# llm-d-incubation/workload-variant-autoscaler

Measured on AMD Instinct MI355X. Metric: solver_wall_clock_ms, lower is better.
Workload: dtype fp64; 1 GPU; model=3 models x 2 service classes (config #3), variants=64, accelerator_types=3, global_batch=64, seq_len=0, parallelism=fleet-shard dp1, analyzer_device=cuda

## Files before the change

### wva_amd/csrc/queue_core.h

```cpp
#pragma once

#include <cmath>

#if defined(__HIPCC__)
#define WVA_HD __host__ __device__ inline
#else
#define WVA_HD inline
#endif

namespace wva {

constexpr double kEpsilon = 0.001;
constexpr double kStabilityFraction = 0.1;
constexpr double kTolerance = 1e-6;
constexpr int kMaxIterations = 100;
constexpr int kMaxQueueToBatchRatio = 10;

enum ProblemField {
  P_ALPHA = 0,
  P_BETA,
  P_GAMMA,
  P_DELTA,
  P_IN_TOKENS,
  P_OUT_TOKENS,
  P_MAX_BATCH,
  P_TARGET_TTFT,
  P_TARGET_ITL,
  P_TARGET_TPS,
  P_TOTAL_RATE,
  P_MIN_REPLICAS,
  PROBLEM_FIELDS
};

enum ResultField {
  R_FEASIBLE = 0,
  R_REPLICAS,
  R_RATE_STAR,
  R_ITL,
  R_TTFT,
  R_RHO,
  RESULT_FIELDS
};

struct Parms {
  double alpha, beta, gamma, delta;
  double in_tokens;
  int out_tokens;
  int max_batch;
  int num_decode;
  double wait_scale;
};

constexpr int kMaxBatchLimit = 2147483647 / (1 + kMaxQueueToBatchRatio);

WVA_HD bool row_valid(const double *pr, double scv = 1.0) {
  bool ok = (scv >= 0.0) & (scv <= 1.7976931348623157e308);
  for (int f = 0; f < PROBLEM_FIELDS; ++f) {
    ok &= fabs(pr[f]) <= 1.7976931348623157e308;
  }
  ok &= (pr[P_ALPHA] >= 0.0) & (pr[P_BETA] >= 0.0) & (pr[P_GAMMA] >= 0.0) &
        (pr[P_DELTA] >= 0.0);
  ok &= (pr[P_MAX_BATCH] >= 1.0) & (pr[P_MAX_BATCH] < (double)kMaxBatchLimit + 1.0);
  ok &= (pr[P_OUT_TOKENS] >= 1.0) & (pr[P_OUT_TOKENS] < 2147483648.0);
  ok &= pr[P_IN_TOKENS] >= 0.0;
  ok &= (pr[P_TARGET_TTFT] >= 0.0) & (pr[P_TARGET_ITL] >= 0.0) & (pr[P_TARGET_TPS] >= 0.0);
  return ok;
}

WVA_HD Parms parms_from_problem(const double *pr, double scv = 1.0) {
  Parms p;
  p.alpha = pr[P_ALPHA];
  p.beta = pr[P_BETA];
  p.gamma = pr[P_GAMMA];
  p.delta = pr[P_DELTA];
  p.in_tokens = trunc(pr[P_IN_TOKENS]);
  p.out_tokens = (int)pr[P_OUT_TOKENS];
  p.max_batch = (int)pr[P_MAX_BATCH];
  p.num_decode = p.out_tokens - 1;
  if (p.in_tokens == 0.0 && p.out_tokens == 1) p.num_decode = 1;
  p.wait_scale = (1.0 + scv) / 2.0;
  return p;
}

WVA_HD int row_chain_length(const double *pr) {
  return row_valid(pr) ? (int)pr[P_MAX_BATCH] * (1 + kMaxQueueToBatchRatio) : 0;
}

WVA_HD double prefill_time(const Parms &p, double batch) {
  return p.in_tokens == 0.0 ? 0.0 : p.gamma + p.delta * p.in_tokens * batch;
}

WVA_HD double decode_time(const Parms &p, double batch) {
  return p.alpha + p.beta * batch;
}

WVA_HD double serv_rate(const Parms &p, int b) {
  return (double)b / (prefill_time(p, (double)b) + p.num_decode * decode_time(p, (double)b));
}

WVA_HD double log_mu(const Parms &p, int n) {
  int b = n + 1;
  if (b > p.max_batch) b = p.max_batch;
  return log(serv_rate(p, b));
}

WVA_HD bool within_tolerance(double x, double value, double tolerance) {
  if (x == value) return true;
  if (value == 0.0 || tolerance < 0.0) return false;
  return fabs((x - value) / value) <= tolerance;
}

WVA_HD double effective_concurrency(const Parms &p, double avg_serv_time) {
  double tokens = (double)(p.out_tokens - 1);
  double numer = avg_serv_time - (p.gamma + p.alpha * tokens);
  double denom = p.delta * p.in_tokens + p.beta * tokens;
  if (denom == 0.0) return numer > 0.0 ? (double)p.max_batch : 0.0;
  double n = numer / denom;
  if (n < 0.0) n = 0.0;
  if (n > (double)p.max_batch) n = (double)p.max_batch;
  return n;
}

struct Stats {
  double throughput;
  double wait;
  double serv;
  double n_serv;
};

WVA_HD bool rate_below(const Parms &p, int b, double lam) {
  double t = prefill_time(p, (double)b) + p.num_decode * decode_time(p, (double)b);
  return (double)b < lam * t;
}

WVA_HD int log_mode_state(const Parms &p, int K, double lam) {
  double tN = prefill_time(p, (double)p.max_batch) +
              p.num_decode * decode_time(p, (double)p.max_batch);
  if ((double)p.max_batch <= lam * tN) return K;
  double t1 = prefill_time(p, 1.0) + p.num_decode * decode_time(p, 1.0);
  if (lam * t1 <= 1.0) return 0;
  int lo = 1, hi = p.max_batch;
  while (lo < hi) {
    int mid = (lo + hi) / 2;
    if (rate_below(p, mid, lam)) {
      lo = mid + 1;
    } else {
      hi = mid;
    }
  }
  return lo - 1;
}

WVA_HD double log_p(const double *cum, double loglam, int n) {
  return (n == 0) ? 0.0 : n * loglam - cum[n - 1];
}

constexpr double kLogCutoff = 45.0;

WVA_HD void state_window(const double *cum, double loglam, int K, int n_star,
                         double m, int *lo_out, int *hi_out) {
  const double thresh = m - kLogCutoff;
  int lo = 0, hi = n_star;
  while (lo < hi) {
    int mid = (lo + hi) / 2;
    if (log_p(cum, loglam, mid) < thresh) {
      lo = mid + 1;
    } else {
      hi = mid;
    }
  }
  *lo_out = lo;
  lo = n_star;
  hi = K;
  while (lo < hi) {
    int mid = (lo + hi + 1) / 2;
    if (log_p(cum, loglam, mid) < thresh) {
      hi = mid - 1;
    } else {
      lo = mid;
    }
  }
  *hi_out = lo;
}

struct GeoTail {
  double S, Ni, eK;
  bool used;
};

WVA_HD GeoTail geo_tail(double x_a, double d, int g_start, int n_hi, int K) {
  GeoTail t{0.0, 0.0, 0.0, false};
  const int M = n_hi - g_start;
  if (M < 8 || fabs(d) * (double)(M + 1) < 0.01) return t;
  const double p_a = exp(x_a);
  const double e1 = expm1(d);
  const double G0 = expm1((double)(M + 1) * d) / e1;
  const double r = e1 + 1.0;
  const double rM = exp((double)M * d);
  const double G1 =
      r * (1.0 - (double)(M + 1) * rM + (double)M * rM * r) / (e1 * e1);
  t.S = p_a * G0;
  t.Ni = p_a * ((double)g_start * G0 + G1);
  if (n_hi == K) t.eK = p_a * exp((double)(K - g_start) * d);
  t.used = true;
  return t;
}

WVA_HD Stats stats_of_sums(double lam, int num, double S, double Ni, double Snum,
                           double Ninum, double eK) {
  Stats st;
  st.throughput = lam * (1.0 - eK / S);
  double n_sys = Ni / S;
  st.n_serv = Ninum / S + (1.0 - Snum / S) * (double)num;
  if (st.throughput == 0.0) {
    st.wait = st.serv = 0.0;
  } else {
    double resp = n_sys / st.throughput;
    st.serv = st.n_serv / st.throughput;
    st.wait = resp - st.serv;
    if (st.wait < 0.0) st.wait = 0.0;
  }
  return st;
}

WVA_HD Stats eval_model(const Parms &p, const double *cum, int K, double lam) {
  double loglam = log(lam);
  int n_star = log_mode_state(p, K, lam);
  double m = log_p(cum, loglam, n_star);
  if (m < 0.0) m = 0.0;
  int n_lo, n_hi;
  state_window(cum, loglam, K, n_star, m, &n_lo, &n_hi);
  int num = p.max_batch;
  double S = 0.0, Ni = 0.0, Snum = 0.0, Ninum = 0.0, eK = 0.0;
  const int g_start = (num + 1 > n_lo) ? num + 1 : n_lo;
  GeoTail tail{0.0, 0.0, 0.0, false};
  int loop_hi = n_hi;
  if (g_start + 8 <= n_hi) {
    const double d = loglam - (cum[g_start] - cum[g_start - 1]);
    tail = geo_tail(log_p(cum, loglam, g_start) - m, d, g_start, n_hi, K);
    if (tail.used) loop_hi = g_start - 1;
  }
  for (int n = n_lo; n <= loop_hi; ++n) {
    double e = exp(log_p(cum, loglam, n) - m);
    S += e;
    Ni += n * e;
    if (n <= num) {
      Snum += e;
      Ninum += n * e;
    }
    if (n == K) eK = e;
  }
  S += tail.S;
  Ni += tail.Ni;
  eK += tail.eK;
  return stats_of_sums(lam, num, S, Ni, Snum, Ninum, eK);
}


WVA_HD double cum_at(const double *cum, int N, double log_mu_n, int n) {
  const int i = n < N ? n : N - 1;
  const double base = cum[i];
  return n < N ? base : base + (double)(n - N + 1) * log_mu_n;
}

WVA_HD double log_p_compact(const double *cum, int N, double log_mu_n, double loglam,
                            int n) {
  return (n == 0) ? 0.0 : n * loglam - cum_at(cum, N, log_mu_n, n - 1);
}

WVA_HD GeoTail geo_tail_compact(const double *cum, int N, double log_mu_n, double loglam,
                                double m, int *loop_hi) {
  const int K = N * (1 + kMaxQueueToBatchRatio);
  const int g_start = N + 1;
  const double d = loglam - log_mu_n;
  const GeoTail tail = geo_tail(
      log_p_compact(cum, N, log_mu_n, loglam, g_start) - m, d, g_start, K, K);
  *loop_hi = tail.used ? N : K;
  return tail;
}

WVA_HD Stats eval_model_compact(const Parms &p, const double *cum, double log_mu_n,
                                double lam) {
  const int num = p.max_batch;
  const int K = num * (1 + kMaxQueueToBatchRatio);
  const double loglam = log(lam);
  const int n_star = log_mode_state(p, K, lam);
  double m = log_p_compact(cum, num, log_mu_n, loglam, n_star);
  if (m < 0.0) m = 0.0;
  int loop_hi;
  const GeoTail tail = geo_tail_compact(cum, num, log_mu_n, loglam, m, &loop_hi);
  double S = 0.0, Ni = 0.0, Snum = 0.0, Ninum = 0.0, eK = 0.0;
  for (int n = 0; n <= loop_hi; ++n) {
    double e = exp(log_p_compact(cum, num, log_mu_n, loglam, n) - m);
    S += e;
    Ni += n * e;
    if (n <= num) {
      Snum += e;
      Ninum += n * e;
    }
    if (n == K) eK = e;
  }
  S += tail.S;
  Ni += tail.Ni;
  eK += tail.eK;
  return stats_of_sums(lam, num, S, Ni, Snum, Ninum, eK);
}

WVA_HD double eval_ttft_of(const Parms &p, const Stats &st) {
  double effc = effective_concurrency(p, st.serv);
  return st.wait * p.wait_scale + prefill_time(p, effc);
}

WVA_HD double eval_itl_of(const Parms &p, const Stats &st) {
  double effc = effective_concurrency(p, st.serv);
  return decode_time(p, effc);
}


constexpr int kBisect = 2;

WVA_HD int classify_bracket(double x_min, double x_max, double y0, double y1,
                            double y_target, double *x_star, bool *increasing) {
  if (within_tolerance(y0, y_target, kTolerance)) {
    *x_star = x_min;
    return 0;
  }
  if (within_tolerance(y1, y_target, kTolerance)) {
    *x_star = x_max;
    return 0;
  }
  if (within_tolerance(y0, y1, kTolerance)) {
    if (y_target > fmax(y0, y1)) {
      *x_star = x_max;
      return +1;
    }
    *x_star = x_min;
    return -1;
  }
  *increasing = y0 < y1;
  if ((*increasing && y_target < y0) || (!*increasing && y_target > y0)) {
    *x_star = x_min;
    return -1;
  }
  if ((*increasing && y_target > y1) || (!*increasing && y_target < y1)) {
    *x_star = x_max;
    return +1;
  }
  return kBisect;
}

template <typename F>
WVA_HD int binary_search(double x_min, double x_max, double y_target, F eval,
                         double *x_star) {
  const double y0 = eval(x_min);
  const double y1 = eval(x_max);
  bool increasing = false;
  const int ind = classify_bracket(x_min, x_max, y0, y1, y_target, x_star, &increasing);
  if (ind != kBisect) return ind;
  double xs = x_min;
  for (int i = 0; i < kMaxIterations; ++i) {
    xs = 0.5 * (x_min + x_max);
    double ys = eval(xs);
    if (within_tolerance(ys, y_target, kTolerance)) break;
    if ((increasing && y_target < ys) || (!increasing && y_target > ys)) {
      x_max = xs;
    } else {
      x_min = xs;
    }
  }
  *x_star = xs;
  return 0;
}


WVA_HD void rate_bracket(const Parms &p, double *lam_min, double *lam_max) {
  *lam_min = serv_rate(p, 1) * kEpsilon;
  *lam_max = serv_rate(p, p.max_batch) * (1.0 - kEpsilon);
}

template <typename Ev>
WVA_HD bool search_targets(const double *pr, const Parms &p, const Ev &ev, double lam_min,
                           double lam_max, double *lam_ttft, double *lam_itl) {
  *lam_ttft = lam_max;
  if (pr[P_TARGET_TTFT] > 0.0) {
    auto ttft = [&](double lam) { return eval_ttft_of(p, ev.eval(lam)); };
    if (binary_search(lam_min, lam_max, pr[P_TARGET_TTFT], ttft, lam_ttft) < 0) return false;
  }
  *lam_itl = lam_max;
  if (pr[P_TARGET_ITL] > 0.0) {
    auto itl = [&](double lam) { return eval_itl_of(p, ev.eval(lam)); };
    if (binary_search(lam_min, lam_max, pr[P_TARGET_ITL], itl, lam_itl) < 0) return false;
  }
  return true;
}

struct RowValues {
  double feasible, replicas, rate_star, itl, ttft, rho;
};

template <typename Ev>
WVA_HD RowValues row_tail(const double *pr, const Parms &p, const Ev &ev, double lam_max,
                          double lam_ttft, double lam_itl) {
  double lam_tps = lam_max;
  if (pr[P_TARGET_TPS] > 0.0) lam_tps = lam_max * (1.0 - kStabilityFraction);

  const double lam = fmin(lam_ttft, fmin(lam_itl, lam_tps));
  Stats st = ev.eval(lam);
  const double rate_star = st.throughput * 1000.0;

  const double total_rate = pr[P_TOTAL_RATE];
  double n_rep = ceil(total_rate / rate_star);
  const double min_rep = trunc(pr[P_MIN_REPLICAS]);
  if (n_rep < min_rep) n_rep = min_rep;
  if (!(n_rep > 0.0)) return RowValues{};
  const double rate = total_rate / n_rep;
  if (!(rate > 0.0) || rate > lam_max * 1000.0) return RowValues{};

  Stats fin = ev.eval(rate / 1000.0);
  double rho = fin.n_serv / (double)p.max_batch;
  rho = fmin(fmax(rho, 0.0), 1.0);

  return RowValues{1.0, n_rep, rate_star, eval_itl_of(p, fin), eval_ttft_of(p, fin), rho};
}

template <typename Ev>
WVA_HD RowValues solve_row(const double *pr, const Parms &p, const Ev &ev) {
  double lam_min, lam_max, lam_ttft, lam_itl;
  rate_bracket(p, &lam_min, &lam_max);
  if (!search_targets(pr, p, ev, lam_min, lam_max, &lam_ttft, &lam_itl)) return RowValues{};
  return row_tail(pr, p, ev, lam_max, lam_ttft, lam_itl);
}

}
```

### wva_amd/csrc/queue_solver_hip.hip

```cpp

#include <hip/hip_runtime.h>

#include "queue_core.h"

namespace wva {



template <typename Pred>
__device__ inline int wave_lower_bound(int lo, int hi, int lane, Pred pred) {
  while (hi - lo >= 64) {
    const int step = (hi - lo + 63) >> 6;
    const int i = lo + lane * step;
    const bool t = (i >= hi) ? true : pred(i);
    const unsigned long long mask = __ballot(t);
    if (mask == 0ull) {
      lo = lo + 63 * step + 1;
      continue;
    }
    const int first = __ffsll((long long)mask) - 1;
    if (first == 0) return lo;
    lo = lo + (first - 1) * step + 1;
    const int cap = lo - 1 + step;
    if (cap < hi) hi = cap;
  }
  const int i = lo + lane;
  const bool t = (i >= hi) ? true : pred(i);
  const unsigned long long mask = __ballot(t);
  return lo + __ffsll((long long)mask) - 1;
}


struct LdsFullTable {
  const double *cum;
  int K;
  static __device__ bool fits(const double *pr, int max_k) {
    return row_chain_length(pr) <= max_k;
  }
  __device__ LdsFullTable(const Parms &p, const double *table)
      : cum(table), K(p.max_batch * (1 + kMaxQueueToBatchRatio)) {}
  __device__ int scan_length() const { return K; }
  __device__ int chain() const { return K; }
  __device__ double log_p(double loglam, int n) const { return wva::log_p(cum, loglam, n); }
  __device__ GeoTail tail(int num, double loglam, double m, int *loop_hi) const {
    const int g_start = num + 1;
    GeoTail t{0.0, 0.0, 0.0, false};
    *loop_hi = K;
    if (g_start + 8 <= K) {
      const double d = loglam - (cum[g_start] - cum[g_start - 1]);
      t = geo_tail(log_p(loglam, g_start) - m, d, g_start, K, K);
      if (t.used) *loop_hi = g_start - 1;
    }
    return t;
  }
};

struct LdsCompactTable {
  const double *cum;
  int N;
  double log_mu_n;
  static __device__ bool fits(const double *pr, int max_n) {
    return trunc(pr[P_MAX_BATCH]) <= (double)max_n;
  }
  __device__ LdsCompactTable(const Parms &p, const double *table)
      : cum(table), N(p.max_batch), log_mu_n(log_mu(p, p.max_batch - 1)) {}
  __device__ int scan_length() const { return N; }
  __device__ int chain() const { return N * (1 + kMaxQueueToBatchRatio); }
  __device__ double log_p(double loglam, int n) const {
    return log_p_compact(cum, N, log_mu_n, loglam, n);
  }
  __device__ GeoTail tail(int, double loglam, double m, int *loop_hi) const {
    return geo_tail_compact(cum, N, log_mu_n, loglam, m, loop_hi);
  }
};

template <int THREADS, typename Table>
struct WgEval {
  static constexpr int WAVES = THREADS / 64;
  const Parms &p;
  Table table;
  double *red;

  __device__ int mode_state_wave(int K, double lam, int lane) const {
    double tN = prefill_time(p, (double)p.max_batch) +
                p.num_decode * decode_time(p, (double)p.max_batch);
    if ((double)p.max_batch <= lam * tN) return K;
    double t1 = prefill_time(p, 1.0) + p.num_decode * decode_time(p, 1.0);
    if (lam * t1 <= 1.0) return 0;
    const int b = wave_lower_bound(
        1, p.max_batch, lane, [&](int i) { return !rate_below(p, i, lam); });
    return b - 1;
  }

  __device__ Stats eval(double lam) const {
    const int tid = threadIdx.x;
    const int wave = tid >> 6;
    const int lane = tid & 63;
    const int K = table.chain();
    const double loglam = log(lam);

    int n_star;
    if constexpr (WAVES == 1) {
      n_star = mode_state_wave(K, lam, lane);
    } else {
      n_star = log_mode_state(p, K, lam);
    }
    double m = table.log_p(loglam, n_star);
    if (m < 0.0) m = 0.0;
    if constexpr (WAVES > 1) {
      __syncthreads();
    }

    const int num = p.max_batch;
    const int idx = (WAVES == 1) ? lane : tid;
    int loop_hi;
    const GeoTail tail = table.tail(num, loglam, m, &loop_hi);
    double S = 0.0, Ni = 0.0, Snum = 0.0, Ninum = 0.0, eK = 0.0;
    {
      double S1 = 0.0, Ni1 = 0.0, Snum1 = 0.0, Ninum1 = 0.0, eK1 = 0.0;
      int n = idx;
      for (; n + THREADS <= loop_hi; n += 2 * THREADS) {
        const int n2 = n + THREADS;
        const double e = exp(table.log_p(loglam, n) - m);
        const double e2 = exp(table.log_p(loglam, n2) - m);
        S += e;
        Ni += (double)n * e;
        S1 += e2;
        Ni1 += (double)n2 * e2;
        if (n <= num) {
          Snum += e;
          Ninum += (double)n * e;
        }
        if (n2 <= num) {
          Snum1 += e2;
          Ninum1 += (double)n2 * e2;
        }
        if (n == K) eK = e;
        if (n2 == K) eK1 = e2;
      }
      if (n <= loop_hi) {
        const double e = exp(table.log_p(loglam, n) - m);
        S += e;
        Ni += (double)n * e;
        if (n <= num) {
          Snum += e;
          Ninum += (double)n * e;
        }
        if (n == K) eK = e;
      }
      S += S1;
      Ni += Ni1;
      Snum += Snum1;
      Ninum += Ninum1;
      eK += eK1;
    }
    for (int off = 32; off > 0; off >>= 1) {
      S += __shfl_down(S, off, 64);
      Ni += __shfl_down(Ni, off, 64);
      Snum += __shfl_down(Snum, off, 64);
      Ninum += __shfl_down(Ninum, off, 64);
      eK += __shfl_down(eK, off, 64);
    }
    if constexpr (WAVES == 1) {
      S = __shfl(S, 0, 64);
      Ni = __shfl(Ni, 0, 64);
      Snum = __shfl(Snum, 0, 64);
      Ninum = __shfl(Ninum, 0, 64);
      eK = __shfl(eK, 0, 64);
    } else {
      if (lane == 0) {
        red[wave * 5 + 0] = S;
        red[wave * 5 + 1] = Ni;
        red[wave * 5 + 2] = Snum;
        red[wave * 5 + 3] = Ninum;
        red[wave * 5 + 4] = eK;
      }
      __syncthreads();
      S = Ni = Snum = Ninum = eK = 0.0;
      for (int w = 0; w < WAVES; ++w) {
        S += red[w * 5 + 0];
        Ni += red[w * 5 + 1];
        Snum += red[w * 5 + 2];
        Ninum += red[w * 5 + 3];
        eK += red[w * 5 + 4];
      }
    }
    S += tail.S;
    Ni += tail.Ni;
    eK += tail.eK;
    return stats_of_sums(lam, num, S, Ni, Snum, Ninum, eK);
  }
};

__device__ inline double row_scv(const double *scv, int pid) {
  return scv != nullptr ? scv[pid] : 1.0;
}

template <typename Table>
__device__ inline bool row_rejected(const double *pr, double scv, int reserved) {
  return !(row_valid(pr, scv) & Table::fits(pr, reserved));
}

__device__ inline void zero_row(double *res) {
  if (threadIdx.x < RESULT_FIELDS) res[threadIdx.x] = 0.0;
}

__device__ inline void store_row(double *res, const RowValues vals) {
  const int tid = threadIdx.x;
  if (tid < RESULT_FIELDS) {
    double v = vals.feasible;
    v = (tid == R_REPLICAS) ? vals.replicas : v;
    v = (tid == R_RATE_STAR) ? vals.rate_star : v;
    v = (tid == R_ITL) ? vals.itl : v;
    v = (tid == R_TTFT) ? vals.ttft : v;
    v = (tid == R_RHO) ? vals.rho : v;
    res[tid] = v;
  }
}

template <int THREADS>
__device__ void build_cum(const Parms &p, int K, double *cum, double *totals) {
  const int tid = threadIdx.x;
  const int chunk = (K + THREADS - 1) / THREADS;
  const int lo = tid * chunk;
  const int hi = min(lo + chunk, K);
  double acc = 0.0;
  for (int n = lo; n < hi; ++n) {
    acc += log_mu(p, n);
    cum[n] = acc;
  }
  totals[tid] = (lo < K) ? acc : 0.0;
  __syncthreads();
  double offset = 0.0;
  for (int t = 0; t < tid; ++t) offset += totals[t];
  for (int n = lo; n < hi; ++n) cum[n] += offset;
  __syncthreads();
}

template <int THREADS, typename Table>
__device__ void solve_body(const double *__restrict__ prob,
                           const double *__restrict__ scv, double *__restrict__ out,
                           int n_problems, int reserved) {
  const int pid = blockIdx.x;
  if (pid >= n_problems) return;
  const double *pr = prob + (size_t)pid * PROBLEM_FIELDS;
  double *res = out + (size_t)pid * RESULT_FIELDS;

  const double cs2 = row_scv(scv, pid);
  zero_row(res);
  if (row_rejected<Table>(pr, cs2, reserved)) return;
  const Parms p = parms_from_problem(pr, cs2);

  extern __shared__ double smem[];
  double *cum = smem;
  double *totals = smem + reserved;
  double *red = totals + THREADS;

  const Table table(p, cum);
  build_cum<THREADS>(p, table.scan_length(), cum, totals);

  WgEval<THREADS, Table> ev{p, table, red};
  store_row(res, solve_row(pr, p, ev));
}

template <typename F>
__device__ int wg_binary_search(double x_min, double x_max, double y_target, F eval,
                                double *x_star) {
  double y0 = eval(x_min);
  if (within_tolerance(y0, y_target, kTolerance)) {
    *x_star = x_min;
    return 0;
  }
  double y1 = eval(x_max);
  if (within_tolerance(y1, y_target, kTolerance)) {
    *x_star = x_max;
    return 0;
  }
  if (within_tolerance(y0, y1, kTolerance)) {
    if (y_target > fmax(y0, y1)) {
      *x_star = x_max;
      return +1;
    }
    *x_star = x_min;
    return -1;
  }
  bool increasing = y0 < y1;
  if ((increasing && y_target < y0) || (!increasing && y_target > y0)) {
    *x_star = x_min;
    return -1;
  }
  if ((increasing && y_target > y1) || (!increasing && y_target < y1)) {
    *x_star = x_max;
    return +1;
  }
  double xs = x_min;
  for (int i = 0; i < kMaxIterations; ++i) {
    xs = 0.5 * (x_min + x_max);
    double ys = eval(xs);
    if (within_tolerance(ys, y_target, kTolerance)) break;
    if ((increasing && y_target < ys) || (!increasing && y_target > ys)) {
      x_max = xs;
    } else {
      x_min = xs;
    }
  }
  *x_star = xs;
  return 0;
}

__device__ void solve_body_dual(const double *__restrict__ prob,
                                const double *__restrict__ scv,
                                double *__restrict__ out, int n_problems, int max_k) {
  constexpr int THREADS = 128;
  const int pid = blockIdx.x;
  if (pid >= n_problems) return;
  const double *pr = prob + (size_t)pid * PROBLEM_FIELDS;
  double *res = out + (size_t)pid * RESULT_FIELDS;
  const int tid = threadIdx.x;
  const int wave = tid >> 6;

  const double cs2 = row_scv(scv, pid);
  zero_row(res);
  if (row_rejected<LdsFullTable>(pr, cs2, max_k)) return;
  const Parms p = parms_from_problem(pr, cs2);

  extern __shared__ double smem[];
  double *cum = smem;
  double *totals = smem + max_k;
  double *ex = totals + THREADS;

  const LdsFullTable table(p, cum);
  build_cum<THREADS>(p, table.scan_length(), cum, totals);

  double lam_min, lam_max;
  rate_bracket(p, &lam_min, &lam_max);

  WgEval<64, LdsFullTable> ev{p, table, nullptr};

  double lam_t = lam_max;
  int ind = 0;
  if (wave == 0) {
    if (pr[P_TARGET_TTFT] > 0.0) {
      ind = wg_binary_search(
          lam_min, lam_max, pr[P_TARGET_TTFT],
          [&](double x) { return eval_ttft_of(p, ev.eval(x)); }, &lam_t);
    }
  } else {
    if (pr[P_TARGET_ITL] > 0.0) {
      ind = wg_binary_search(
          lam_min, lam_max, pr[P_TARGET_ITL],
          [&](double x) { return eval_itl_of(p, ev.eval(x)); }, &lam_t);
    }
  }
  if ((tid & 63) == 0) {
    ex[wave * 2 + 0] = lam_t;
    ex[wave * 2 + 1] = (double)ind;
  }
  __syncthreads();
  if (ex[1] < 0.0 || ex[3] < 0.0) return;
  if (wave == 1) return;

  store_row(res, row_tail(pr, p, ev, lam_max, ex[0], ex[2]));
}


__device__ inline void mb_publish(volatile double *slot, double y,
                                  volatile double *flag, double round_id) {
  *slot = y;
  __threadfence_block();
  *flag = round_id;
}

constexpr unsigned kMailboxSpinLimit = 1u << 24;

__device__ inline bool mb_wait(volatile double *flags, int n, double round_id) {
  for (int j = 0; j < n; ++j) {
    unsigned spins = 0;
    while (flags[j] < round_id) {
      __builtin_amdgcn_s_sleep(2);
      if (++spins > kMailboxSpinLimit) return false;
    }
  }
  __threadfence_block();
  return true;
}

__device__ inline double heap_midpoint(double lo, double hi, int k) {
  double x = 0.5 * (lo + hi);
  const int depth_below = 31 - __clz(k);
  for (int level = depth_below - 1; level >= 0; --level) {
    if ((k >> level) & 1) {
      lo = x;
    } else {
      hi = x;
    }
    x = 0.5 * (lo + hi);
  }
  return x;
}

template <int D, typename F>
__device__ int spec_binary_search(double x_min, double x_max, double y_target,
                                  F eval, int sub, volatile double *yb,
                                  volatile double *fl, double *x_star) {
  constexpr int SW = (1 << D) - 1;
  const int lane = threadIdx.x & 63;

  double mine = 0.0;
  if (sub == 0) mine = eval(x_min);
  if (sub == 1) mine = eval(x_max);
  if (lane == 0 && sub < 2) mb_publish(&yb[sub], mine, &fl[sub], 1.0);
  if (!mb_wait(fl, 2, 1.0)) {
    *x_star = x_min;
    return -1;
  }
  const double y0 = yb[0];
  const double y1 = yb[1];
  bool increasing = false;
  const int cls = classify_bracket(x_min, x_max, y0, y1, y_target, x_star, &increasing);
  if (cls != kBisect) return cls;

  double lo = x_min, hi = x_max, xs = x_min;
  double round_id = 2.0;
  int iters = 0;
  while (iters < kMaxIterations) {
    const double x_mine = heap_midpoint(lo, hi, sub + 1);
    const double y_mine = eval(x_mine);
    if (lane == 0) mb_publish(&yb[sub], y_mine, &fl[sub], round_id);
    if (!mb_wait(fl, SW, round_id)) {
      *x_star = x_min;
      return -1;
    }
    round_id += 1.0;

    int k = 1;
    bool done = false;
    for (int level = 0; level < D && iters < kMaxIterations; ++level) {
      xs = 0.5 * (lo + hi);
      const double ys = yb[k - 1];
      ++iters;
      if (within_tolerance(ys, y_target, kTolerance)) {
        done = true;
        break;
      }
      if ((increasing && y_target < ys) || (!increasing && y_target > ys)) {
        hi = xs;
        k = 2 * k;
      } else {
        lo = xs;
        k = 2 * k + 1;
      }
    }
    if (done) break;
  }
  *x_star = xs;
  return 0;
}

template <int D>
__device__ void solve_body_spec(const double *__restrict__ prob,
                                const double *__restrict__ scv,
                                double *__restrict__ out, int n_problems,
                                int max_k) {
  constexpr int SW = (1 << D) - 1;
  constexpr int THREADS = 2 * SW * 64;
  const int pid = blockIdx.x;
  if (pid >= n_problems) return;
  const double *pr = prob + (size_t)pid * PROBLEM_FIELDS;
  double *res = out + (size_t)pid * RESULT_FIELDS;
  const int tid = threadIdx.x;
  const int wave = tid >> 6;
  const int group = wave / SW;
  const int sub = wave % SW;
  const int lane = tid & 63;

  const double cs2 = row_scv(scv, pid);
  zero_row(res);
  if (row_rejected<LdsFullTable>(pr, cs2, max_k)) return;
  const Parms p0 = parms_from_problem(pr, cs2);

  extern __shared__ double smem[];
  double *cum = smem;
  double *totals = smem + max_k;
  double *mail = totals + THREADS;
  if (tid < 34) mail[tid] = 0.0;
  static_assert(sizeof(Parms) <= 8 * sizeof(double), "Parms outgrew its LDS slot");
  const Parms *pp = &p0;
  if constexpr (D == 3) {
    Parms *shared_parms = reinterpret_cast<Parms *>(mail + 40);
    if (tid == 0) *shared_parms = p0;
    pp = shared_parms;
  }

  const LdsFullTable table(p0, cum);
  build_cum<THREADS>(p0, table.scan_length(), cum, totals);
  const Parms &p = *pp;

  double lam_min, lam_max;
  rate_bracket(p, &lam_min, &lam_max);

  WgEval<64, LdsFullTable> ev{p, table, nullptr};

  volatile double *yb = mail + group * 14;
  volatile double *fl = yb + 7;
  volatile double *ex = mail + 28;
  volatile double *done = mail + 32;

  double lam_t = lam_max;
  int ind = 0;
  const double target = (group == 0) ? pr[P_TARGET_TTFT] : pr[P_TARGET_ITL];
  if (target > 0.0) {
    if (group == 0) {
      ind = spec_binary_search<D>(
          lam_min, lam_max, target,
          [&](double x) { return eval_ttft_of(p, ev.eval(x)); }, sub, yb, fl, &lam_t);
    } else {
      ind = spec_binary_search<D>(
          lam_min, lam_max, target,
          [&](double x) { return eval_itl_of(p, ev.eval(x)); }, sub, yb, fl, &lam_t);
    }
  }
  if (sub == 0 && lane == 0) {
    ex[group * 2 + 0] = lam_t;
    ex[group * 2 + 1] = (double)ind;
    __threadfence_block();
    done[group] = 1.0;
  }
  if (wave != 0) return;

  if (!mb_wait(done, 2, 1.0)) return;
  if (ex[1] < 0.0 || ex[3] < 0.0) return;

  store_row(res, row_tail(pr, p, ev, lam_max, ex[0], ex[2]));
}

extern "C" __global__ void __launch_bounds__(384) wva_solve_kernel_384(
    const double *__restrict__ prob, const double *__restrict__ scv,
    double *__restrict__ out, int n_problems, int max_k) {
  solve_body_spec<2>(prob, scv, out, n_problems, max_k);
}

extern "C" __global__ void __launch_bounds__(896) wva_solve_kernel_896(
    const double *__restrict__ prob, const double *__restrict__ scv,
    double *__restrict__ out, int n_problems, int max_k) {
  solve_body_spec<3>(prob, scv, out, n_problems, max_k);
}

extern "C" __global__ void __launch_bounds__(256) wva_solve_kernel_256(
    const double *__restrict__ prob, const double *__restrict__ scv,
    double *__restrict__ out, int n_problems, int max_k) {
  solve_body<256, LdsFullTable>(prob, scv, out, n_problems, max_k);
}

extern "C" __global__ void __launch_bounds__(64) wva_solve_kernel_64(
    const double *__restrict__ prob, const double *__restrict__ scv,
    double *__restrict__ out, int n_problems, int max_k) {
  solve_body<64, LdsFullTable>(prob, scv, out, n_problems, max_k);
}

extern "C" __global__ void __launch_bounds__(128) wva_solve_kernel_128(
    const double *__restrict__ prob, const double *__restrict__ scv,
    double *__restrict__ out, int n_problems, int max_k) {
  solve_body_dual(prob, scv, out, n_problems, max_k);
}

constexpr int kCompactThreads = 256;

extern "C" __global__ void __launch_bounds__(kCompactThreads) wva_solve_kernel_compact(
    const double *__restrict__ prob, const double *__restrict__ scv,
    double *__restrict__ out, int n_problems, int max_n) {
  solve_body<kCompactThreads, LdsCompactTable>(prob, scv, out, n_problems, max_n);
}

}

#include <cstdlib>
#include <cstring>

namespace {

using SizingKernel = void (*)(const double *, const double *, double *, int, int);

struct Geometry {
  int threads;
  const char *name;
  SizingKernel kernel;
};

enum { kSeq64, kDual128, kSeq256, kSpec384, kSpec896 };

const Geometry kGeometries[] = {
    {64, "64", wva::wva_solve_kernel_64},    {128, "128", wva::wva_solve_kernel_128},
    {256, "256", wva::wva_solve_kernel_256}, {384, "384", wva::wva_solve_kernel_384},
    {896, "896", wva::wva_solve_kernel_896},
};

bool fits_lds(int table_len, int threads) {
  return table_len <= 64 * 1024 / 8 - threads - 64;
}

int launch(const Geometry &g, const double *prob, const double *scv, double *out,
           int n_problems, int table_len, void *stream) {
  if (table_len < 1 || !fits_lds(table_len, g.threads)) return -1;
  const size_t smem = (size_t)(table_len + g.threads + 64) * sizeof(double);
  hipLaunchKernelGGL(g.kernel, dim3(n_problems), dim3(g.threads), smem, (hipStream_t)stream,
                     prob, scv, out, n_problems, table_len);
  return (int)hipGetLastError();
}

}

extern "C" int wva_launch_solve_scv(const double *prob, const double *scv, double *out,
                                    int n_problems, int max_k, void *stream) {
  const Geometry *g = nullptr;
  if (const char *env = std::getenv("WVA_GPU_THREADS")) {
    for (const Geometry &listed : kGeometries) {
      if (std::strcmp(env, listed.name) == 0) g = &listed;
    }
  }
  if (g != nullptr && g->threads > 256 && !fits_lds(max_k, g->threads)) g = nullptr;
  if (g == nullptr) {
    g = &kGeometries[n_problems >= 512 ? kDual128 : fits_lds(max_k, 384) ? kSpec384 : kSeq256];
  }
  return launch(*g, prob, scv, out, n_problems, max_k, stream);
}

extern "C" int wva_launch_solve_compact(const double *prob, const double *scv, double *out,
                                        int n_problems, int max_n, void *stream) {
  const Geometry compact{wva::kCompactThreads, "", wva::wva_solve_kernel_compact};
  return launch(compact, prob, scv, out, n_problems, max_n, stream);
}
```

Measured before the change: 829.2 us.

## Dedupe log_mu in prefix scan and reuse search throughput in row tail

```diff
diff --git a/wva_amd/csrc/queue_core.h b/wva_amd/csrc/queue_core.h
--- a/wva_amd/csrc/queue_core.h
+++ b/wva_amd/csrc/queue_core.h
@@ -102,6 +102,42 @@
   int b = n + 1;
   if (b > p.max_batch) b = p.max_batch;
   return log(serv_rate(p, b));
+}
+
+
+WVA_HD int scan_distinct(const Parms &p, int K) { return p.max_batch < K ? p.max_batch : K; }
+
+WVA_HD void scan_fill_logs(const Parms &p, int K, int tid, int threads, double *cum,
+                           double *log_mu_n) {
+  const int distinct = scan_distinct(p, K);
+  for (int n = tid; n < distinct; n += threads) {
+    const double l = log_mu(p, n);
+    cum[n] = l;
+    if (n == p.max_batch - 1) *log_mu_n = l;
+  }
+}
+
+WVA_HD double scan_part(const Parms &p, int K, int part, int parts, double *cum,
+                        double log_mu_n) {
+  const int distinct = scan_distinct(p, K);
+  const int chunk = (K + parts - 1) / parts;
+  const int lo = part * chunk;
+  const int hi = lo + chunk < K ? lo + chunk : K;
+  double acc = 0.0;
+  for (int n = lo; n < hi; ++n) {
+    acc += (n < distinct) ? cum[n] : log_mu_n;
+    cum[n] = acc;
+  }
+  return lo < K ? acc : 0.0;
+}
+
+WVA_HD void scan_offset_part(int K, int part, int parts, const double *totals, double *cum) {
+  const int chunk = (K + parts - 1) / parts;
+  const int lo = part * chunk;
+  const int hi = lo + chunk < K ? lo + chunk : K;
+  double offset = 0.0;
+  for (int t = 0; t < part; ++t) offset += totals[t];
+  for (int n = lo; n < hi; ++n) cum[n] += offset;
 }
 
 WVA_HD bool within_tolerance(double x, double value, double tolerance) {
@@ -398,15 +434,33 @@
   double feasible, replicas, rate_star, itl, ttft, rho;
 };
 
+struct KnownRate {
+  double lam, throughput;
+  bool valid;
+};
+
+WVA_HD KnownRate known_rate(bool has_ttft, double lam_ttft, double thr_ttft, bool has_itl,
+                            double lam_itl, double thr_itl) {
+  if (has_itl && (!has_ttft || lam_itl < lam_ttft)) return KnownRate{lam_itl, thr_itl, true};
+  if (has_ttft) return KnownRate{lam_ttft, thr_ttft, true};
+  return KnownRate{0.0, 0.0, false};
+}
+
 template <typename Ev>
 WVA_HD RowValues row_tail(const double *pr, const Parms &p, const Ev &ev, double lam_max,
-                          double lam_ttft, double lam_itl) {
+                          double lam_ttft, double lam_itl,
+                          const KnownRate known = KnownRate{0.0, 0.0, false}) {
   double lam_tps = lam_max;
   if (pr[P_TARGET_TPS] > 0.0) lam_tps = lam_max * (1.0 - kStabilityFraction);
 
   const double lam = fmin(lam_ttft, fmin(lam_itl, lam_tps));
-  Stats st = ev.eval(lam);
-  const double rate_star = st.throughput * 1000.0;
+  double throughput;
+  if (known.valid && lam == known.lam) {
+    throughput = known.throughput;
+  } else {
+    throughput = ev.eval(lam).throughput;
+  }
+  const double rate_star = throughput * 1000.0;
 
   const double total_rate = pr[P_TOTAL_RATE];
   double n_rep = ceil(total_rate / rate_star);
diff --git a/wva_amd/csrc/queue_solver_hip.hip b/wva_amd/csrc/queue_solver_hip.hip
--- a/wva_amd/csrc/queue_solver_hip.hip
+++ b/wva_amd/csrc/queue_solver_hip.hip
@@ -218,22 +218,17 @@
   }
 }
 
+constexpr int kScanSlackSlot = 63;
+
 template <int THREADS>
 __device__ void build_cum(const Parms &p, int K, double *cum, double *totals) {
   const int tid = threadIdx.x;
-  const int chunk = (K + THREADS - 1) / THREADS;
-  const int lo = tid * chunk;
-  const int hi = min(lo + chunk, K);
-  double acc = 0.0;
-  for (int n = lo; n < hi; ++n) {
-    acc += log_mu(p, n);
-    cum[n] = acc;
-  }
-  totals[tid] = (lo < K) ? acc : 0.0;
+  double *log_mu_n = totals + THREADS + kScanSlackSlot;
+  scan_fill_logs(p, K, tid, THREADS, cum, log_mu_n);
   __syncthreads();
-  double offset = 0.0;
-  for (int t = 0; t < tid; ++t) offset += totals[t];
-  for (int n = lo; n < hi; ++n) cum[n] += offset;
+  totals[tid] = scan_part(p, K, tid, THREADS, cum, *log_mu_n);
+  __syncthreads();
+  scan_offset_part(K, tid, THREADS, totals, cum);
   __syncthreads();
 }
 
@@ -338,29 +333,43 @@
   WgEval<64, LdsFullTable> ev{p, table, nullptr};
 
   double lam_t = lam_max;
+  double thr_t = 0.0;
   int ind = 0;
   if (wave == 0) {
     if (pr[P_TARGET_TTFT] > 0.0) {
       ind = wg_binary_search(
           lam_min, lam_max, pr[P_TARGET_TTFT],
-          [&](double x) { return eval_ttft_of(p, ev.eval(x)); }, &lam_t);
+          [&](double x) {
+            const Stats st = ev.eval(x);
+            thr_t = st.throughput;
+            return eval_ttft_of(p, st);
+          },
+          &lam_t);
     }
   } else {
     if (pr[P_TARGET_ITL] > 0.0) {
       ind = wg_binary_search(
           lam_min, lam_max, pr[P_TARGET_ITL],
-          [&](double x) { return eval_itl_of(p, ev.eval(x)); }, &lam_t);
+          [&](double x) {
+            const Stats st = ev.eval(x);
+            thr_t = st.throughput;
+            return eval_itl_of(p, st);
+          },
+          &lam_t);
     }
   }
   if ((tid & 63) == 0) {
     ex[wave * 2 + 0] = lam_t;
     ex[wave * 2 + 1] = (double)ind;
+    ex[4 + wave] = thr_t;
   }
   __syncthreads();
   if (ex[1] < 0.0 || ex[3] < 0.0) return;
   if (wave == 1) return;
 
-  store_row(res, row_tail(pr, p, ev, lam_max, ex[0], ex[2]));
+  const KnownRate known = known_rate(pr[P_TARGET_TTFT] > 0.0, ex[0], ex[4],
+                                     pr[P_TARGET_ITL] > 0.0, ex[2], ex[5]);
+  store_row(res, row_tail(pr, p, ev, lam_max, ex[0], ex[2], known));
 }
 
 
@@ -402,7 +411,8 @@
 template <int D, typename F>
 __device__ int spec_binary_search(double x_min, double x_max, double y_target,
                                   F eval, int sub, volatile double *yb,
-                                  volatile double *fl, double *x_star) {
+                                  volatile double *tb, volatile double *fl,
+                                  double *x_star, double *thr_star) {
   constexpr int SW = (1 << D) - 1;
   const int lane = threadIdx.x & 63;
 
@@ -418,7 +428,10 @@
   const double y1 = yb[1];
   bool increasing = false;
   const int cls = classify_bracket(x_min, x_max, y0, y1, y_target, x_star, &increasing);
-  if (cls != kBisect) return cls;
+  if (cls != kBisect) {
+    *thr_star = tb[*x_star == x_max ? 1 : 0];
+    return cls;
+  }
 
   double lo = x_min, hi = x_max, xs = x_min;
   double round_id = 2.0;
@@ -451,11 +464,16 @@
         k = 2 * k + 1;
       }
     }
-    if (done) break;
+    if (done || iters >= kMaxIterations) {
+      *thr_star = tb[(done ? k : k >> 1) - 1];
+      break;
+    }
   }
   *x_star = xs;
   return 0;
 }
+
+constexpr int kThroughputSlots = 42;
 
 template <int D>
 __device__ void solve_body_spec(const double *__restrict__ prob,
@@ -487,7 +505,7 @@
   static_assert(sizeof(Parms) <= 8 * sizeof(double), "Parms outgrew its LDS slot");
   const Parms *pp = &p0;
   if constexpr (D == 3) {
-    Parms *shared_parms = reinterpret_cast<Parms *>(mail + 40);
+    Parms *shared_parms = reinterpret_cast<Parms *>(mail + 34);
     if (tid == 0) *shared_parms = p0;
     pp = shared_parms;
   }
@@ -503,26 +521,40 @@
 
   volatile double *yb = mail + group * 14;
   volatile double *fl = yb + 7;
+  volatile double *tb = yb + kThroughputSlots;
   volatile double *ex = mail + 28;
   volatile double *done = mail + 32;
+  volatile double *ex_thr = mail + 49;
 
   double lam_t = lam_max;
+  double thr_t = 0.0;
   int ind = 0;
   const double target = (group == 0) ? pr[P_TARGET_TTFT] : pr[P_TARGET_ITL];
   if (target > 0.0) {
     if (group == 0) {
       ind = spec_binary_search<D>(
           lam_min, lam_max, target,
-          [&](double x) { return eval_ttft_of(p, ev.eval(x)); }, sub, yb, fl, &lam_t);
+          [&](double x) {
+            const Stats st = ev.eval(x);
+            if (lane == 0) tb[sub] = st.throughput;
+            return eval_ttft_of(p, st);
+          },
+          sub, yb, tb, fl, &lam_t, &thr_t);
     } else {
       ind = spec_binary_search<D>(
           lam_min, lam_max, target,
-          [&](double x) { return eval_itl_of(p, ev.eval(x)); }, sub, yb, fl, &lam_t);
+          [&](double x) {
+            const Stats st = ev.eval(x);
+            if (lane == 0) tb[sub] = st.throughput;
+            return eval_itl_of(p, st);
+          },
+          sub, yb, tb, fl, &lam_t, &thr_t);
     }
   }
   if (sub == 0 && lane == 0) {
     ex[group * 2 + 0] = lam_t;
     ex[group * 2 + 1] = (double)ind;
+    ex_thr[group] = thr_t;
     __threadfence_block();
     done[group] = 1.0;
   }
@@ -531,7 +563,9 @@
   if (!mb_wait(done, 2, 1.0)) return;
   if (ex[1] < 0.0 || ex[3] < 0.0) return;
 
-  store_row(res, row_tail(pr, p, ev, lam_max, ex[0], ex[2]));
+  const KnownRate known = known_rate(pr[P_TARGET_TTFT] > 0.0, ex[0], ex_thr[0],
+                                     pr[P_TARGET_ITL] > 0.0, ex[2], ex_thr[1]);
+  store_row(res, row_tail(pr, p, ev, lam_max, ex[0], ex[2], known));
 }
 
 extern "C" __global__ void __launch_bounds__(384) wva_solve_kernel_384(
```

New measurement: 831.3 us. No clear change (+0.3%).
